# bioinformatics-centre/kaiju

Measured on AMD Instinct MI355X. Metric: classified reads/sec (150 bp), higher is better.
Workload: dtype u64

## Files before the change

kaiju_amd/csrc/capi.hip:

```cpp
#include <hip/hip_runtime.h>
#include <fcntl.h>
#include <sys/stat.h>
#include <time.h>
#include <unistd.h>

#include <algorithm>
#include <atomic>
#include <cstdio>
#include <cstring>
#include <future>
#include <memory>
#include <mutex>
#include <stdexcept>
#include <string>
#include <thread>
#include <vector>
#include <chrono>

#include "../../include/kaiju_gpu.h"
#include "fmi_stream.h"
#include "host_index.h"
#include "host_tables.h"
#include "kj_core.h"
#include "taxonomy.h"
// ... 65 lines not shown

constexpr int kS1TeamBlock = 256;
constexpr int kS1TeamsPerBlock = kS1TeamBlock / (int)kS1TeamLanes;
__global__ void __launch_bounds__(kS1TeamBlock)
k_fragments_team(const Stage1Tables *__restrict__ g_t, Params p, Batch b, uint32_t *err) {
  __shared__ __attribute__((aligned(16))) Stage1Tables s_t;
  __shared__ __attribute__((aligned(16))) S1TeamLds s_team[kS1TeamsPerBlock];
  {
    const uint4 *src = reinterpret_cast<const uint4 *>(g_t);
    uint4 *dst = reinterpret_cast<uint4 *>(&s_t);
    for (uint32_t i = threadIdx.x; i < sizeof(Stage1Tables) / 16; i += kS1TeamBlock) dst[i] = src[i];
    __syncthreads();
  }
  const uint32_t team = threadIdx.x / kS1TeamLanes;
  const uint32_t r = blockIdx.x * kS1TeamsPerBlock + team;
  if (r >= b.n_reads) return;
  uint32_t e = 0;
  S1TeamDev tm{&s_team[team], threadIdx.x % kS1TeamLanes};
  build_fragments_team(s_t, p, b, r, &e, tm);
  if (e) atomicOr(err, e);
}

__global__ void __launch_bounds__(256)
k_trigcheck(const Stage1Tables *__restrict__ g_t, Params p, Batch b, uint32_t *seglist, uint32_t *segcount) {
  __shared__ __attribute__((aligned(16))) Stage1Tables s_t;
  __shared__ __attribute__((aligned(4))) uint8_t s_cnt[256 * kS1CntStride];
  {
    const uint4 *src = reinterpret_cast<const uint4 *>(g_t);
    uint4 *dst = reinterpret_cast<uint4 *>(&s_t);
    for (uint32_t i = threadIdx.x; i < sizeof(Stage1Tables) / 16; i += 256) dst[i] = src[i];
    __syncthreads();
  }
  const uint32_t r = blockIdx.x * 256 + threadIdx.x;
  if (r >= b.n_reads) return;
  const uint32_t v = b.hits[r].reserved;
  if (v == 0) return;
  b.hits[r].reserved = 0;
  const bool need = lazy_seg_needed(s_t, p, b, r, b.hits + r, v, nullptr, s_cnt + threadIdx.x * kS1CntStride);
  if (need) seglist[atomicAdd(segcount, 1u)] = r;
}
__global__ void __launch_bounds__(256)
k_segflag(Params p, SegTables st, Batch b, SegQueue sq, const uint32_t *seglist, const uint32_t *segcount, uint32_t *err) {
  __shared__ int64_t s_entg[13];
  if (threadIdx.x < 13) s_entg[threadIdx.x] = st.ent_g[threadIdx.x];
  __syncthreads();
  const SegCtx cx = seg_ctx(st, s_entg, nullptr);
  const uint32_t n = *segcount;
  for (uint32_t i = blockIdx.x * 256 + threadIdx.x; i < n; i += gridDim.x * 256) {
    const uint32_t r = seglist[i];
    const ReadMeta rm = b.meta[r];
    Frag *F = b.frags + rm.frag;
    const uint8_t *pep = b.pep + rm.pep;
    const uint32_t nf = rm.nfrag & ~kNfragSegPending;
    uint32_t pending = 0;
    for (uint32_t k = 0; k < nf; k++) {
      const Frag f = F[k];
      uint32_t fl = kFragChecked;
      if (seg_triggers(cx, pep + f.start, (int)f.len)) {
        const uint32_t slot = atomicAdd(sq.count, 1u);
        if (slot >= sq.cap) atomicOr(err, 2u);
        else {
          SegWork wk; wk.read = r; wk.frag = k;
          sq.items[slot] = wk;
          pending = kNfragSegPending;
          fl = (slot + 1) << kFragSlotShift;
        }
      }
      F[k].flags = fl;
    }
    b.meta[r].nfrag = nf | pending;
    uint64_t *h8 = reinterpret_cast<uint64_t *>(b.hits + r);
    for (int x = 0; x < (int)(sizeof(Hit) / 8); x++) h8[x] = 0;
  }
}
__global__ void __launch_bounds__(kBlock)
k_seg_apply_list(const ConstTables *__restrict__ g_ct, Params p, Batch b, SegQueue sq, const uint32_t *seglist,
                 const uint32_t *segcount, uint32_t *err) {
  __shared__ ConstTables s_ct;
  load_tables(s_ct, g_ct);
  const uint32_t n = *segcount;
  uint32_t e = 0;
  for (uint32_t i = blockIdx.x * kBlock + threadIdx.x; i < n; i += gridDim.x * kBlock) seg_apply_mem(s_ct, p, b, sq, seglist[i], &e);
  if (e) atomicOr(err, e);
}

#ifdef KJ_POST_WAVES
#define KJ_POST_BOUNDS __launch_bounds__(256, KJ_POST_WAVES)
#else
#define KJ_POST_BOUNDS __launch_bounds__(256)
#endif
template <bool LCA>
__global__ void KJ_POST_BOUNDS
k_mem_post1(const Stage1Tables *__restrict__ g_t, DevIndex ix, Params p, Batch b, DevTaxonomy t, CompactHit *__restrict__ compact, int lazy,
            uint32_t *seglist, uint32_t *segcount, uint32_t *todo, uint32_t *todocount) {
  __shared__ __attribute__((aligned(16))) Stage1Tables s_t;
  __shared__ __attribute__((aligned(4))) uint8_t s_cnt[256 * kS1CntStride];
  if (lazy) {
    const uint4 *src = reinterpret_cast<const uint4 *>(g_t);
    uint4 *dst = reinterpret_cast<uint4 *>(&s_t);
    for (uint32_t i = threadIdx.x; i < sizeof(Stage1Tables) / 16; i += 256) dst[i] = src[i];
    __syncthreads();
  }
  const uint32_t r = blockIdx.x * 256 + threadIdx.x;
  bool need = false, later = false;
  if (r < b.n_reads) {
    Hit *h = b.hits + r;
    const uint32_t v = lazy ? h->reserved : 0u;
    if (v != 0) {
      h->reserved = 0;
#ifndef KJ_POST_NOTRIG
      need = lazy_seg_needed(s_t, p, b, r, h, v, nullptr, s_cnt + threadIdx.x * kS1CntStride);
#endif
    }
    if (!need) {
      if (h->flags & kHitRetry) later = true;
#ifdef KJ_POST_NOLOCATE
      else if (LCA) { CompactHit ch; ch.lca = 0; ch.best = h->best; ch.info = 0; compact[r] = ch; }
#else
      else if (!mem_locate_read<false>(ix, p, h, kLocDeferRows)) later = true;
      else if (LCA) compact[r] = compact_hit(t, *h);
#endif
    }
  }
  const uint32_t lane = threadIdx.x & 63u;
  {
    const uint64_t m = __ballot(need);
    if (m) {
      const uint32_t leader = (uint32_t)__builtin_ctzll(m);
      uint32_t base = 0;
      if (lane == leader) base = atomicAdd(segcount, (uint32_t)__popcll(m));
      base = (uint32_t)__shfl((int)base, (int)leader, 64);
      if (need) seglist[base + (uint32_t)__popcll(m & ((1ull << lane) - 1ull))] = r;
    }
  }
// ... 1501 lines not shown
  Params kp{};
  hipStream_t stream = nullptr;
  hipEvent_t ev[6] = {nullptr, nullptr, nullptr, nullptr, nullptr, nullptr};
  bool ev_valid = false;
  int n_cu = 0, blocks_main = 0, blocks_retry = 0;
  DevBuf pep, frags, meta, counters, retry_list, seg_items, seg_recs;
  DevBuf scratch_main[10], scratch_retry[5], h_compact;
  DevBuf redo_bitmap, redo_list, redo_items, redo_index, redo_pool, redo_work, redo_cls;
  bool greedy2 = false;
  bool greedy3 = false;
  uint32_t g3_split = 1;
  uint32_t g3_threads = 512;
  uint32_t g1_pool = 192, g1_match = 64;
  bool g1_pool_set = false;
  uint32_t greedy_gate = 1u | 32u << 8;
  bool verbose = false;
  bool exact_pass = true;
  bool count_ops = false;
  bool mem_v1 = false;
  bool verbose_v1 = false;
  bool stage1_old = false;
  bool stage1_lane = false;
  bool lazy_seg = true;
  DevBuf seglist, loc_list, todo_list;
  int seg_team = 64;
  bool fused_post = true;
  const char *dump_frags = nullptr;
  uint32_t vb_text_cap = 0;
  DevBuf vb_nacc, vb_acc, vb_tlen, vb_text, vb_bestv, vb_bestv_retry;
  DevBuf vb_packed, vb_pos;
  std::vector<uint8_t> vb_host;
  std::vector<uint32_t> vb_h_nacc, vb_h_acc;
  DevBuf h_seqs, h_off, h_hits;
  kj_ingest_scratch *ingest = nullptr;
  DevBuf ing_text1, ing_text2, ing_names, ing_info;
  kaiju_gpu_stats stats{};
  uint32_t last_n = 0;
  uint32_t max_read_len = 1024;
  ~kaiju_gpu_ctx() {
    if (!ix) return;
    (void)hipSetDevice(ix->device);
    if (ingest) kj_ingest_free(ingest);
    DevBuf *all[] = {&ing_text1, &ing_text2, &ing_names, &ing_info, &pep, &frags, &meta, &counters, &retry_list, &seg_items, &seg_recs, &h_seqs, &h_off, &h_hits, &h_compact, &seglist, &loc_list, &todo_list,
                     &vb_nacc, &vb_acc, &vb_tlen, &vb_text, &vb_bestv, &vb_bestv_retry, &vb_packed, &vb_pos,
                     &redo_bitmap, &redo_list, &redo_items, &redo_index, &redo_pool, &redo_work, &redo_cls};
    for (DevBuf *b : all) if (b->p) (void)hipFree(b->p);
// ... 33 lines not shown
  if (!out || !ix || !p) return fail(KAIJU_GPU_ERR_ARG, "NULL argument");
  *out = nullptr;
  if (p->mode != 0 && p->mode != 1) return fail(KAIJU_GPU_ERR_ARG, "mode must be 0 (MEM) or 1 (GREEDY)");
  if (p->min_fragment_length < 1 || p->min_fragment_length > 10000)
    return fail(KAIJU_GPU_ERR_UNSUPPORTED, "min_fragment_length out of range");
  if (p->mode == 1 && p->mismatches > (uint32_t)kMaxMismatch)
    return fail(KAIJU_GPU_ERR_UNSUPPORTED, "more than 8 mismatches are not supported");
  if (p->mode == 1 && p->seed_length < 1) return fail(KAIJU_GPU_ERR_ARG, "seed_length must be >= 1");
  if (p->max_match_ids > 20 || p->max_matches_SI > 64 || p->max_matches_SI < 1)
    return fail(KAIJU_GPU_ERR_UNSUPPORTED, "max_match_ids <= 20 and 1 <= max_matches_SI <= 64 required");
  std::unique_ptr<kaiju_gpu_ctx> c(new kaiju_gpu_ctx());
  c->ix = ix;
  c->params = *p;
  c->kp.mode = p->mode; c->kp.m = p->min_fragment_length; c->kp.mismatches = p->mismatches;
  c->kp.min_score = p->min_score; c->kp.seed_length = p->seed_length; c->kp.seg = p->seg ? 1 : 0;
  c->kp.max_matches_SI = p->max_matches_SI; c->kp.max_match_ids = p->max_match_ids;
  if (const char *e = getenv("KAIJU_GPU_DEBUG")) c->kp.debug = (uint32_t)atoi(e);
  if (const char *e = getenv("KAIJU_GPU_EXACT_PASS")) c->exact_pass = atoi(e) != 0;
  if (const char *e = getenv("KAIJU_GPU_MEM_LANE")) c->mem_v1 = !strcmp(e, "v1");
  if (const char *e = getenv("KAIJU_GPU_VERBOSE_LANE")) c->verbose_v1 = !strcmp(e, "v1");
  c->dump_frags = getenv("KAIJU_GPU_DUMP_FRAGS");
  if (const char *e = getenv("KAIJU_GPU_STAGE1")) { c->stage1_old = !strcmp(e, "old"); c->stage1_lane = !strcmp(e, "lane"); }
  if (const char *e = getenv("KAIJU_GPU_LAZY_SEG")) c->lazy_seg = atoi(e) != 0;
  if (const char *e = getenv("KAIJU_GPU_FUSED_POST")) c->fused_post = atoi(e) != 0;
  if (const char *e = getenv("KAIJU_GPU_SEG_TEAM")) { const int v = atoi(e); if (v == 8 || v == 16 || v == 32 || v == 64) c->seg_team = v; }
  if (ix->id_mode == KAIJU_GPU_IDS_SEQUENCE && p->mode == 0) c->kp.flags |= kParamXOrder;
  if (p->input_is_protein) c->kp.flags |= kParamProtein;
  KJ_HIP(hipSetDevice(ix->device));
  hipDeviceProp_t prop;
  KJ_HIP(hipGetDeviceProperties(&prop, ix->device));
  c->n_cu = prop.multiProcessorCount;
  int occ = 0;
  if (p->mode == 0) KJ_HIP(hipOccupancyMaxActiveBlocksPerMultiprocessor(&occ, k_mem, kBlock, 0));
  else {
    const bool g_wide = ix->dev.mb_base != nullptr;
    const uint32_t g_k = g_wide ? ix->dev.kmer_k : ix->dev.kline_k;
    c->greedy2 = ix->dev.blocks64 && (g_wide ? ix->dev.kmer64 != nullptr : ix->dev.kline != nullptr) && g_k >= 2 &&
                 g_k <= p->seed_length && p->seed_length >= 3;
    if (const char *e = getenv("KAIJU_GPU_GREEDY_LANE")) { if (!strcmp(e, "v1")) c->greedy2 = false; }
#ifdef KJ_GREEDY3
    if (const char *e = getenv("KAIJU_GPU_GREEDY_LANE")) { if (!strcmp(e, "v3")) c->greedy3 = c->greedy2 && !g_wide; }
    if (const char *e = getenv("KAIJU_GPU_G3_SPLIT")) c->g3_split = (uint32_t)atoi(e);
    if (const char *e = getenv("KAIJU_GPU_G3_THREADS")) { const int v = atoi(e); if (v >= 64 && v <= kG3Threads && v % 64 == 0) c->g3_threads = (uint32_t)v; }
#else
    if (const char *e = getenv("KAIJU_GPU_GREEDY_LANE")) {
      if (!strcmp(e, "v3")) return fail(KAIJU_GPU_ERR_UNSUPPORTED, "KAIJU_GPU_GREEDY_LANE=v3: this library was built without -DKJ_GREEDY3 (tests/tools/mem_variants.sh, variant g3)");
// ... 196 lines not shown
      const bool xo = (p.flags & kParamXOrder) != 0;
      SIEntry *si_main = static_cast<SIEntry *>(c->scratch_main[0].p);
      auto launch_v2 = [&](const Params &pp, const WorkList &wl, bool counting, bool second = false) {
        if (c->verbose) {
          if (mem_narrow2) hipLaunchKernelGGL(k_mem_vb, dim3(c->blocks_main), blk, 0, s, ix->dev, pp, b, wl, si_main, si_cap, vb.acc);
          else hipLaunchKernelGGL(k_mem_wide2_vb, dim3(c->blocks_main), blk, 0, s, ix->dev, pp, b, wl, si_main, si_cap, vb.acc);
        } else
        if (mem_narrow2) {
          if (second && !xo) hipLaunchKernelGGL(k_mem_second, dim3(c->blocks_main), blk, 0, s, ix->dev, pp, b, wl, si_main, si_cap);
          else if (counting) hipLaunchKernelGGL(k_mem_count, dim3(c->blocks_main), blk, 0, s, ix->dev, pp, b, wl, si_main, si_cap);
          else if (xo) hipLaunchKernelGGL(k_mem_x, dim3(c->blocks_main), blk, 0, s, ix->dev, pp, b, wl, si_main, si_cap);
          else hipLaunchKernelGGL(k_mem, dim3(c->blocks_main), blk, 0, s, ix->dev, pp, b, wl, si_main, si_cap);
        } else {
          if (counting) hipLaunchKernelGGL(k_mem_wide2_count, dim3(c->blocks_main), blk, 0, s, ix->dev, pp, b, wl, si_main, si_cap);
          else if (xo) hipLaunchKernelGGL(k_mem_wide2_x, dim3(c->blocks_main), blk, 0, s, ix->dev, pp, b, wl, si_main, si_cap);
          else hipLaunchKernelGGL(k_mem_wide2, dim3(c->blocks_main), blk, 0, s, ix->dev, pp, b, wl, si_main, si_cap);
        }
      };
      const bool defer = mem_v2;
      Params pd = p;
      if (defer) pd.flags |= kParamDeferLocate;
      if (mem_v2) {
        Params pm = pd;
        if (lazy) pm.flags |= kParamLazySeg;
        launch_v2(pm, wl_main, c->count_ops);
      } else if (!ix->dev.mb_base)
        hipLaunchKernelGGL(k_mem_v1, dim3(c->blocks_main), blk, 0, s, ix->dev, p, b, wl_main, si_main, si_cap, vb);
      else
        hipLaunchKernelGGL(k_mem_wide, dim3(c->blocks_main), blk, 0, s, ix->dev, p, b, wl_main, si_main, si_cap, vb);
      KJ_HIP(hipGetLastError());
      KJ_HIP(hipEventRecord(c->ev[3], s));
      uint32_t *todo = nullptr;
      const DevTaxonomy dt = tax ? tax->dev : DevTaxonomy{};
      CompactHit *const cmp = reinterpret_cast<CompactHit *>(d_compact);
      if (fused) {
        if ((rc = ensure(c->seglist, (size_t)n * 4 + 16))) return rc;
        if ((rc = ensure(c->todo_list, (size_t)n * 4 + 16))) return rc;
        todo = static_cast<uint32_t *>(c->todo_list.p);
        uint32_t *seglist = static_cast<uint32_t *>(c->seglist.p);
        if (tax) hipLaunchKernelGGL(k_mem_post1<true>, grid_reads, dim3(256), 0, s, ix->d_s1, ix->dev, p, b, dt, cmp, lazy ? 1 : 0, seglist, cnt + 22, todo, cnt + 26);
        else hipLaunchKernelGGL(k_mem_post1<false>, grid_reads, dim3(256), 0, s, ix->d_s1, ix->dev, p, b, dt, cmp, lazy ? 1 : 0, seglist, cnt + 22, todo, cnt + 26);
        KJ_HIP(hipGetLastError());
      }
      if (lazy) {
        if ((rc = ensure(c->seglist, (size_t)n * 4 + 16))) return rc;
        uint32_t *seglist = static_cast<uint32_t *>(c->seglist.p);
        if (!fused) hipLaunchKernelGGL(k_trigcheck, grid_reads, dim3(256), 0, s, ix->d_s1, p, b, seglist, cnt + 22);
        hipLaunchKernelGGL(k_segflag, dim3(c->n_cu * 4), dim3(256), 0, s, p, ix->st, b, sq, seglist, cnt + 22, cnt + 3);
        launch_seg(c, s, p, ix->st, b, sq);
        hipLaunchKernelGGL(k_seg_apply_list, dim3(c->n_cu * 4), blk, 0, s, ix->d_ct, p, b, sq, seglist, cnt + 22, cnt + 3);
        WorkList wl_seg;
        wl_seg.counter = cnt + 23; wl_seg.reads = seglist; wl_seg.n_items_ptr = cnt + 22; wl_seg.n_items = 0;
        wl_seg.retry_list = wl_main.retry_list; wl_seg.retry_count = wl_main.retry_count;
        launch_v2(pd, wl_seg, false, true);
        KJ_HIP(hipGetLastError());
      }
      hipLaunchKernelGGL(k_mem_retry, dim3(blocks_retry), blk, 0, s, ix->dev, p, b, wl_retry,
                         static_cast<SIEntry *>(c->scratch_retry[0].p), si_cap_retry, vb);
      KJ_HIP(hipGetLastError());
      if (defer && c->verbose) {
        if (mem_narrow2) hipLaunchKernelGGL(k_mem_verbose<false>, grid_reads, dim3(256), 0, s, ix->dev, p, b, vb);
        else hipLaunchKernelGGL(k_mem_verbose<true>, grid_reads, dim3(256), 0, s, ix->dev, p, b, vb);
        KJ_HIP(hipGetLastError());
      }
      if (defer && !fused) {
        if (mem_narrow2 && ix->dev.row_tax) {
          hipLaunchKernelGGL(k_mem_locate<false>, grid_reads, dim3(256), 0, s, ix->dev, p, b, loc_list, cnt + 24);
          hipLaunchKernelGGL(k_mem_locate_list<false>, dim3(c->n_cu * 8), dim3(256), 0, s, ix->dev, p, b, loc_list, cnt + 24);
        }
        else if (mem_narrow2) hipLaunchKernelGGL(k_mem_locate_team, grid_team, dim3(256), 0, s, ix->dev, p, b);
        else if (ix->dev.row_tax) {
// ... 755 lines not shown
```

kaiju_amd/csrc/kj_core.h:

```cpp
#pragma once
#include <type_traits>
#include <stdint.h>

#if defined(__HIPCC__)
#include <hip/hip_runtime.h>
#define KJ_HD __host__ __device__ __forceinline__
#define KJ_HD_NOINLINE __host__ __device__ __noinline__
#else
#define KJ_HD inline
#define KJ_HD_NOINLINE inline
struct uint2 { uint32_t x, y; };
struct ulonglong2 { uint64_t x, y; };
#endif

namespace kj {

struct u128 { uint64_t x, y; };
typedef u128 u128_unaligned __attribute__((aligned(1)));
typedef uint32_t u32_unaligned __attribute__((aligned(1)));
typedef uint64_t u64_unaligned __attribute__((aligned(1)));

constexpr int kMaxIds = 21;
constexpr int kSbShift = 16;
constexpr uint32_t kHitIdCap = 1u, kHitSiCap = 2u;
// ... 128 lines not shown
      {d.seq_valid, (uint64_t)d.nseq},
      {d.kmer32 ? (const void *)d.kmer32 : (const void *)d.kmer64, d.kmer_k ? nw * (d.kmer32 ? sizeof(uint2) : sizeof(ulonglong2)) : 0},
      {d.kline, d.kline ? nlw * kKLineBytes : 0},
      {d.text, d.text ? text_bytes : 0},
      {d.sa_full ? (const void *)d.sa_full : (const void *)d.sa_tpos5, d.sa_full ? d.bwtlen * 4 : d.sa_tpos5 ? tpos_bytes : 0},
      {d.row_tax, d.row_tax ? d.bwtlen * 4 : 0},
      {d.tax_of_dense, d.tax_of_dense ? (uint64_t)d.n_dense * 8 : 0}};
  for (int x = 0; x < kIndexArrays; x++) { out[x] = a[x]; if (!out[x].p || !out[x].bytes) out[x] = IndexArr{nullptr, 0}; }
}

struct Params {
  int32_t mode;
  uint32_t m;
  uint32_t mismatches, min_score, seed_length;
  int32_t seg;
  uint32_t max_matches_SI, max_match_ids;
  uint32_t debug = 0;
  uint32_t flags = 0;
};
constexpr uint32_t kParamDeferLocate = 8u;
constexpr uint32_t kParamXOrder = 1u;
constexpr uint32_t kParamProtein = 2u;
constexpr uint32_t kParamLazySeg = 4u;
constexpr uint32_t kWinMulti = 0x80000000u;
constexpr uint32_t kWinForce = 0xffffffffu;

struct Frag {
  uint32_t start;
  uint32_t len;
  uint32_t key;
  uint32_t flags;
};

struct SegWork { uint32_t read, frag; };
constexpr int kSegRecRegions = 15;
struct SegRec {
  uint16_t n;
  uint16_t overflow;
  uint16_t lr[kSegRecRegions][2];
};
static_assert(sizeof(SegRec) == 64, "SegRec is 64 bytes");
struct SegQueue {
  SegWork *items;
  SegRec *recs;
  uint32_t *count;
  uint32_t cap;
};
constexpr uint32_t kFragChecked = 1u, kFragRemoved = 2u, kFragSlotShift = 8;
constexpr uint32_t kNfragSegPending = 0x80000000u;

struct SIEntry {
  uint64_t lo;
  uint32_t len;
  uint32_t frag;
};

struct Hit {
// ... 22 lines not shown
  uint8_t subst_rank[20][20];
  uint8_t codon_idx[64];
};

struct ReadMeta {
  uint64_t pep;
  uint32_t frag;
  uint32_t nfrag;
};

struct Batch {
  const uint8_t *seqs;
  const uint64_t *off;
  uint32_t n_reads;
  int32_t paired;
  uint8_t *pep;
  Frag *frags;
  ReadMeta *meta;
  Hit *hits;
};

constexpr uint64_t kPepPerRead = 208;
static_assert(kPepPerRead >= 2 * 96 + 15 + 1, "kPepPerRead must cover the unit padding of build_fragments_fast plus the rounding of pep_base");
KJ_HD uint64_t pep_base(const uint64_t *off, uint32_t r) { return ((2 * off[2 * (uint64_t)r] + 15) & ~15ull) + kPepPerRead * r + 16; }
KJ_HD uint64_t frag_base(const uint64_t *off, uint32_t r, uint32_t m) {
  return 2 * ((2 * off[2 * (uint64_t)r]) / (m + 1) + 7ull * r);
}
KJ_HD uint32_t frag_cap(const uint64_t *off, uint32_t r, uint32_t m) {
  return (uint32_t)(frag_base(off, r + 1, m) - frag_base(off, r, m));
}

KJ_HD uint32_t popc64(uint64_t x) { return (uint32_t)__builtin_popcountll(x); }

#if defined(__HIP_DEVICE_COMPILE__)
KJ_HD uint64_t kj_ballot(bool p) { return __ballot(p); }
KJ_HD uint32_t kj_lane() { return threadIdx.x & 63u; }
KJ_HD uint32_t kj_bcast(uint32_t v, uint32_t src_lane) { return (uint32_t)__shfl((int)v, (int)src_lane, 64); }
KJ_HD uint32_t kj_rank_below(uint64_t mask) {
  return __builtin_amdgcn_mbcnt_hi((uint32_t)(mask >> 32), __builtin_amdgcn_mbcnt_lo((uint32_t)mask, 0u));
}
KJ_HD uint32_t kj_bcast_uniform(uint32_t v, uint32_t src_lane) {
  return (uint32_t)__builtin_amdgcn_readlane((int)v, (int)__builtin_amdgcn_readfirstlane((int)src_lane));
}
KJ_HD uint32_t kj_alignbyte(uint32_t hi, uint32_t lo, uint32_t s) { return __builtin_amdgcn_alignbyte(hi, lo, s); }
#else
KJ_HD uint32_t kj_alignbyte(uint32_t hi, uint32_t lo, uint32_t s) { return (uint32_t)((((uint64_t)hi << 32) | lo) >> (8u * (s & 3u))); }
KJ_HD uint64_t kj_ballot(bool p) { return p ? 1ull : 0ull; }
// ... 626 lines not shown
    pep.put(base + (uint32_t)g * fcap + nres, 0);
    emit_run(p, list, n, cap, rbase + (uint32_t)g * fcap, R_len[g], R_sum[g], R_pend[g], R_trig[g]);
    pep.put(rbase + (uint32_t)g * fcap + nres, 0);
  }
}

template <class S>
KJ_HD bool seg_triggers(const SegCtx &cx, const S &s, int len) {
  if (len < kSegWindow) return false;
  SegWin w{0, 0, 0};
  segwin_open(w, cx, s, 0);
  if (w.score <= cx.ent_locut) return true;
  for (int start = 0; start + kSegWindow < len; start++) {
    segwin_shift(w, cx, s, start);
    if (w.score <= cx.ent_locut) return true;
  }
  return false;
}

template <class Coop, class Sync>
KJ_HD void seg_compute(const SegCtx &cx, const Coop &coop, const Batch &b, const Params &p, const SegQueue &sq,
                       uint32_t slot, uint8_t *stage, uint32_t stage_cap, int32_t *work, uint8_t *cls, Sync &&team_sync) {
  const SegWork wk = sq.items[slot];
  const ReadMeta rm = b.meta[wk.read];
  const Frag f = b.frags[rm.frag + wk.frag];
  const uint8_t *pep = b.pep + rm.pep;
  const uint8_t *src = pep + f.start;
  if (stage && f.len <= stage_cap) {
    team_sync();
    for (uint32_t x = (uint32_t)coop.lane(); x < f.len; x += (uint32_t)coop.width()) stage[x] = src[x];
    team_sync();
    src = stage;
  }
  int32_t *left = work + 2 * kSegMaxRegions, *right = work + 3 * kSegMaxRegions;
  bool ov = false;
  const int n = seg_regions(cx, coop, src, (int)f.len, left, right, ov, work, (stage && f.len <= stage_cap) ? cls : nullptr, team_sync);
  if (coop.lane() != 0) return;
  SegRec rec;
  rec.overflow = (ov || n > kSegRecRegions || f.len > 65535u) ? 1 : 0;
  rec.n = (uint16_t)(n > kSegRecRegions ? kSegRecRegions : n);
  for (int k = 0; k < kSegRecRegions; k++) {
    rec.lr[k][0] = k < n ? (uint16_t)left[k] : 0;
    rec.lr[k][1] = k < n ? (uint16_t)right[k] : 0;
  }
  sq.recs[slot] = rec;
}

template <class Sink>
KJ_HD void seg_split(const ConstTables &t, const Params &p, const SegRec &rec, const uint8_t *pep,
                     const Frag &f, Sink &&sink) {
// ... 86 lines not shown
  const uint64_t pbase = pep_base(b.off, r);
  PepBuf pep;
  if (stage) { pep.base = stage; pep.row = stage_row; } else { pep.base = b.pep + pbase; pep.row = 4; }
  uint32_t n = 0, pending = 0;
  const bool skip = b.paired ? (len1 < m3 && len2 < m3) : (len1 < m3);
  if (!skip) {
    const uint32_t seq2 = 2 * len1 + 6, seq_end = seq2 + 2 * len2 + 6;
    if (len1 >= m3) translate_mate(t, p, tc, b.seqs + o0, len1, 0, pep, 0, list, n, cap);
    if (b.paired && len2 >= m3) translate_mate(t, p, tc, b.seqs + o1, len2, seq2, pep, 6 * (len1 / 3 + 1), list, n, cap);
    if (stage && !(p.debug & 8u)) {
      const uint32_t used = 6 * (len1 / 3 + 1) + (b.paired ? 6 * (len2 / 3 + 1) : 0);
      u128 *dst = reinterpret_cast<u128 *>(b.pep + pbase);
      for (uint32_t q = 0; q * 16 < used; q++) {
        u128 v;
        v.x = (uint64_t)pep.get32(16 * q) | (uint64_t)pep.get32(16 * q + 4) << 32;
        v.y = (uint64_t)pep.get32(16 * q + 8) | (uint64_t)pep.get32(16 * q + 12) << 32;
        dst[q] = v;
      }
    }
    if (p.debug & 16u) n = 0;
    uint32_t sb = 1;
    while ((1u << sb) <= seq_end) sb++;
    const uint32_t kbound = 11u * ((len1 > len2 ? len1 : len2) / 3u + 1u);
    auto final_flags = [&](uint32_t trig, uint32_t k) -> uint32_t {
      if (!p.seg) return 0u;
      if (!trig) return kFragChecked;
      const uint32_t slot = append_slot(sq.count);
      if (slot >= sq.cap) { if (err_flags) *err_flags |= 2u; return kFragChecked; }
      SegWork wk; wk.read = r; wk.frag = k;
      sq.items[slot] = wk;
      pending = kNfragSegPending;
      return (slot + 1) << kFragSlotShift;
    };
    if (stage && n <= stage_words / 2 && sb <= 20 && kbound < (1u << (31 - sb))) {
      uint32_t *row = reinterpret_cast<uint32_t *>(stage);
      const uint32_t rw = stage_row / 4, half = stage_words / 2, smax = (1u << sb) - 1u;
      for (uint32_t k0 = 0; k0 < n; k0 += 4) {
        Frag f[4];
#pragma unroll
        for (int x = 0; x < 4; x++) f[x] = list[k0 + (uint32_t)x < n ? k0 + (uint32_t)x : k0];
#pragma unroll
        for (int x = 0; x < 4; x++) {
          const uint32_t k = k0 + (uint32_t)x;
          if (k < n) {
            row[(size_t)k * rw] = f[x].key << (sb + 1) | (smax - (f[x].flags >> 1)) << 1 | (f[x].flags & 1u);
            row[(size_t)(half + k) * rw] = f[x].start << 16 | f[x].len;
          }
        }
      }
      for (uint32_t k = 0; k < n; k++) {
        const uint32_t ck = row[(size_t)k * rw];
        uint32_t rank = 0;
        for (uint32_t q = 0; q < n; q++) rank += row[(size_t)q * rw] > ck ? 1u : 0u;
        const uint32_t sl = row[(size_t)(half + k) * rw];
        Frag f; f.start = sl >> 16; f.len = sl & 0xffffu; f.key = ck >> (sb + 1); f.flags = final_flags(ck & 1u, rank);
        list[rank] = f;
      }
    } else {
      for (uint32_t k = 1; k < n; k++) {
        const Frag f = list[k];
        uint32_t pos = k;
        while (pos > 0 && (list[pos - 1].key < f.key || (list[pos - 1].key == f.key && list[pos - 1].flags > f.flags))) {
          list[pos] = list[pos - 1]; pos--;
        }
        list[pos] = f;
      }
      for (uint32_t k = 0; k < n; k++) list[k].flags = final_flags(list[k].flags & 1u, k);
    }
  }
  ReadMeta rm; rm.pep = pbase; rm.frag = (uint32_t)frag_base(b.off, r, p.m); rm.nfrag = n | pending;
  b.meta[r] = rm;
}

struct Stage1Tables {
  uint8_t nuc3[256];
  uint8_t tf[512];
  uint8_t tr[512];
  int32_t dtab[32];
  uint8_t diag[32];
  int32_t locut32;
  int32_t pad[3];
};
static_assert(sizeof(Stage1Tables) % 16 == 0, "Stage1Tables is copied in 16-byte pieces");
constexpr int kS1Units = 4;
constexpr uint32_t kS1MaxLen = 48 * kS1Units - 1;
constexpr int kS1UnitsLong = 6;
constexpr uint32_t kS1MaxLenLong = 48 * kS1UnitsLong - 1;
struct Mask128 { uint64_t lo, hi; };
KJ_HD uint64_t mk_zero(uint64_t) { return 0; }
KJ_HD Mask128 mk_zero(Mask128) { return Mask128{0, 0}; }
KJ_HD void mk_or16(uint64_t &m, uint32_t bits, uint32_t b) { m |= (uint64_t)bits << (16u * b); }
KJ_HD void mk_or16(Mask128 &m, uint32_t bits, uint32_t b) { if (b < 4u) m.lo |= (uint64_t)bits << (16u * b); else m.hi |= (uint64_t)bits << (16u * (b - 4u)); }
KJ_HD void mk_setbit(uint64_t &m, uint32_t k, bool v) { m |= (uint64_t)(v ? 1u : 0u) << k; }
KJ_HD void mk_setbit(Mask128 &m, uint32_t k, bool v) { if (k < 64u) m.lo |= (uint64_t)(v ? 1u : 0u) << k; else m.hi |= (uint64_t)(v ? 1u : 0u) << (k - 64u); }
KJ_HD bool mk_any(uint64_t m) { return m != 0; }
KJ_HD bool mk_any(const Mask128 &m) { return (m.lo | m.hi) != 0; }
KJ_HD uint64_t mk_shr(uint64_t m, uint32_t n) { return m >> n; }
KJ_HD Mask128 mk_shr(const Mask128 &m, uint32_t n) {
  if (n == 0u) return m;
  if (n >= 128u) return Mask128{0, 0};
  if (n >= 64u) return Mask128{m.hi >> (n - 64u), 0};
  return Mask128{(m.lo >> n) | (m.hi << (64u - n)), m.hi >> n};
}
KJ_HD uint64_t mk_shl(uint64_t m, uint32_t n) { return m << n; }
KJ_HD Mask128 mk_shl(const Mask128 &m, uint32_t n) {
  if (n == 0u) return m;
  if (n >= 128u) return Mask128{0, 0};
  if (n >= 64u) return Mask128{0, m.lo << (n - 64u)};
  return Mask128{m.lo << n, (m.hi << n) | (m.lo >> (64u - n))};
}
// ... 195 lines not shown
      sc += same ? 0 : dx - dy;
      any = any || sc <= t.locut32;
    }
#pragma unroll
    for (int q = 0; q < 4; q++) pw[q] = w[q];
  }
  return any;
}
KJ_HD bool lazy_seg_needed(const Stage1Tables &t, const Params &p, const Batch &b, uint32_t r, const Hit *h, uint32_t v, uint8_t *buf, uint8_t *row) {
  if (v == kWinForce) return true;
  const ReadMeta rm = b.meta[r];
  const Frag *F = b.frags + rm.frag;
  const uint8_t *pep = b.pep + rm.pep;
  if (!(v & kWinMulti)) {
    const Frag f = F[(v & ~kWinMulti) - 1u];
    return buf ? trig_fragment(t, pep, f.start, f.len, buf, row) : trig_fragment_units(t, pep, f.start, f.len, row);
  }
  const uint32_t best = h->best, nf = rm.nfrag & ~kNfragSegPending;
  for (uint32_t k = 0; k < nf; k++) {
    const Frag f = F[k];
    if (f.len >= best && (buf ? trig_fragment(t, pep, f.start, f.len, buf, row) : trig_fragment_units(t, pep, f.start, f.len, row))) return true;
  }
  return false;
}
KJ_HD uint64_t bitrev64(uint64_t v) {
#if defined(__HIP_DEVICE_COMPILE__)
  return __brevll(v);
#else
  uint64_t r = 0;
  for (int i = 0; i < 64; i++) r |= ((v >> i) & 1ull) << (63 - i);
  return r;
#endif
}

KJ_HD uint64_t mk_rev_low(uint64_t m, uint32_t nbits) { return bitrev64(m) >> (64u - nbits); }
KJ_HD Mask128 mk_rev_low(const Mask128 &m, uint32_t nbits) { return mk_shr(Mask128{bitrev64(m.hi), bitrev64(m.lo)}, 128u - nbits); }

KJ_HD uint32_t s1_start(int f, uint32_t u, uint32_t a, uint32_t l) {
  return f < 3 ? (uint32_t)f * (16 * u) + a : (uint32_t)(f + 1) * (16 * u) - a - l;
}

template <class MaskT, class Emit>
KJ_HD void s1_runs(const MaskT *ns, const MaskT *tg, uint32_t len, uint32_t m, uint32_t area, uint32_t seq_base,
                   Emit &&emit) {
  if (m > 64u || m == 0u) return;
  const uint32_t top = len - 3, u = len / 48u + 1u;
// ... 69 lines not shown
    MaskT ns[6], tg[6];
    for (int f = 0; f < 6; f++) tg[f] = mk_zero(MaskT{});
    auto scan_mate = [&](uint8_t *dst, uint32_t len) {
      const uint32_t u = len / 48u + 1u;
      for (int f = 0; f < 6; f++) {
        const MaskT mm = trig_scan_units<UNITS, MaskT>(t, dst + (size_t)f * 16 * u, u, ln.cnt);
        const MaskT tv = f < 3 ? mm : mk_shl(mk_rev_low(mm, 16 * u), 11);
#pragma unroll
        for (int q = 0; q < 6; q++) if (q == f) tg[q] = tv;
      }
    };
    if (len1 >= m3) {
      s1_mate(t, b.seqs + o0, len1, area, ns);
#ifndef KJ_S1_NOSCAN
      if (TRIG && p.seg) scan_mate(area, len1);
#endif
      s1_runs(ns, tg, len1, p.m, 0, 0, emit);
    }
    if (b.paired && len2 >= m3) {
      s1_mate(t, b.seqs + o1, len2, area + mate_bytes, ns);
      if (TRIG && p.seg) scan_mate(area + mate_bytes, len2);
      s1_runs(ns, tg, len2, p.m, mate_bytes, 2 * len1 + 6, emit);
    }
    auto final_flags = [&](uint32_t trig, uint32_t k) -> uint32_t {
      if (!TRIG || !p.seg) return 0u;
      if (!trig) return kFragChecked;
      const uint32_t slot = append_slot(sq.count);
      if (slot >= sq.cap) { if (err_flags) *err_flags |= 2u; return kFragChecked; }
      SegWork wk; wk.read = r; wk.frag = k;
      sq.items[slot] = wk;
      pending = kNfragSegPending;
      return (slot + 1) << kFragSlotShift;
    };
    if (n <= (uint32_t)kS1ListCap) {
      for (uint32_t k = 0; k < n; k++) {
        const uint32_t hi = ln.codes[(size_t)(2 * k) * ln.code_stride], lo = ln.codes[(size_t)(2 * k + 1) * ln.code_stride];
        uint32_t rank = 0;
        for (uint32_t q = 0; q < n; q++) rank += ln.codes[(size_t)(2 * q) * ln.code_stride] > hi ? 1u : 0u;
        Frag f; f.start = lo >> 8; f.len = (lo >> 1) & 127u; f.key = hi >> 11; f.flags = final_flags(lo & 1u, rank);
        list[rank] = f;
      }
    } else {
      for (uint32_t k = 0; k < (uint32_t)kS1ListCap; k++) {
        const uint32_t hi = ln.codes[(size_t)(2 * k) * ln.code_stride], lo = ln.codes[(size_t)(2 * k + 1) * ln.code_stride];
        Frag f; f.start = lo >> 8; f.len = (lo >> 1) & 127u; f.key = hi >> 11; f.flags = (2047u - (hi & 2047u)) << 1 | (lo & 1u);
        list[k] = f;
      }
      for (uint32_t k = 1; k < n; k++) {
        const Frag f = list[k];
        uint32_t pos = k;
        while (pos > 0 && (list[pos - 1].key < f.key || (list[pos - 1].key == f.key && list[pos - 1].flags > f.flags))) {
          list[pos] = list[pos - 1]; pos--;
        }
        list[pos] = f;
      }
      for (uint32_t k = 0; k < n; k++) list[k].flags = final_flags(list[k].flags & 1u, k);
    }
  }
  ReadMeta rm; rm.pep = pbase; rm.frag = fbase; rm.nfrag = n | pending;
  b.meta[r] = rm;
}

constexpr uint32_t kS1TeamLanes = 16;
struct S1TeamLds {
  u128 str[6 * kS1Units];
  uint64_t ns[6];
  uint32_t hi[kS1ListCap], lo[kS1ListCap];
  uint32_t n, pad[3];
};
static_assert(sizeof(S1TeamLds) % 16 == 0, "S1TeamLds is an array of 16-byte aligned team areas");

struct S1TeamHost {
  static constexpr int kSlots = (int)kS1TeamLanes;
  S1TeamLds *lds;
  KJ_HD uint32_t lane(int s) const { return (uint32_t)s; }
  KJ_HD void sync() const {}
  KJ_HD void sync_memory() const {}
  KJ_HD uint32_t xor1(const uint32_t *v, int s) const { return v[s ^ 1]; }
  KJ_HD uint32_t dword(const uint8_t *s, uint32_t len, int32_t at) const {
// ... 237 lines not shown
        emit_run(p, list, n, cap, run_start, run_len, sum, seq++, trig);
        run_len = 0; sum = 0; trig = false;
        trig_reset(w);
      }
    }
    *reinterpret_cast<uint64_t *>(pep + (len & ~7u)) = wacc;
    emit_run(p, list, n, cap, run_start, run_len, sum, seq, trig);
    for (uint32_t k = 1; k < n; k++) {
      const Frag f = list[k];
      uint32_t pos = k;
      while (pos > 0 && (list[pos - 1].key < f.key || (list[pos - 1].key == f.key && list[pos - 1].flags > f.flags))) {
        list[pos] = list[pos - 1]; pos--;
      }
      list[pos] = f;
    }
    for (uint32_t k = 0; k < n; k++) {
      uint32_t fl = 0;
      if (p.seg) {
        fl = kFragChecked;
        if (list[k].flags & 1u) {
          const uint32_t slot = append_slot(sq.count);
          if (slot >= sq.cap) { if (err_flags) *err_flags |= 2u; }
          else {
            SegWork wk; wk.read = r; wk.frag = k;
            sq.items[slot] = wk;
            pending = kNfragSegPending;
            fl = (slot + 1) << kFragSlotShift;
          }
        }
      }
      list[k].flags = fl;
    }
  }
  ReadMeta rm; rm.pep = pbase; rm.frag = (uint32_t)frag_base(b.off, r, p.m); rm.nfrag = n | pending;
  b.meta[r] = rm;
}

KJ_HD void seg_apply_mem(const ConstTables &t, const Params &p, const Batch &b, const SegQueue &sq, uint32_t r,
                         uint32_t *err_flags) {
  const ReadMeta rm = b.meta[r];
  const uint32_t raw = rm.nfrag;
  if (!(raw & kNfragSegPending)) return;
  const uint32_t n_orig = raw & ~kNfragSegPending;
  Frag *list = b.frags + rm.frag;
  const uint32_t cap = frag_cap(b.off, r, p.m);
  const uint8_t *pep = b.pep + rm.pep;
  uint32_t np = 0;
  for (uint32_t k = 0; k < n_orig; k++) {
// ... 700 lines not shown
    if (parked) kind = kind_saved;
    KJ_PM(PM_TAIL);
    {
      if (bk == BK_END_MATCH) {
        KJ_PM(PM_END_MATCH);
        const uint32_t l = (uint32_t)(j - i + 1);
        KJ_HIST_SINGLE_END(l);
        if constexpr (kSpanEq) last_sz = hi > lo ? (P)(hi - lo) : (P)1;
        bool probed = false;
        if constexpr (WIDE) {
          if (pj >= 0) {
            probed = true;
            if (l < pw) { j--; pj = -1; }
            else { j = pj; pj = -2; i = flen; }
            bk = BK_START_J;
          }
        }
        if (probed) {}
        else
        if (l >= L) {
          if (l > L) { nsi = 0; ovf = false; L = l; multi = false; }
          const uint32_t ilen = (uint32_t)(int32_t)(hi - lo);
          if (nsi != 0 && fcur != s0frag) multi = true;
          if constexpr (VERBOSE) { if (nsi < (uint32_t)kVbMem) ls.vbm[(size_t)r * kVbAcc + nsi] = fcur << 16 | ((uint32_t)i & 0xffffu); }
          if (nsi == 0) { s0lo = lo; s0len = ilen; s0frag = fcur; }
          else if (nsi == 1) { s1lo = lo; s1len = ilen; s1frag = fcur; }
          else if (nsi < ls.si_cap) { SIEntry e; e.lo = lo; e.len = ilen; e.frag = fcur; ls.si[nsi] = e; if constexpr (COUNT) oc[kOpcSiSpill]++; }
          else ovf = true;
          nsi++;
          found = true;
        }
        if (probed) {}
        else if (i <= 1) bk = BK_NEXT_FRAG;
        else { j--; bk = BK_START_J; }
      }
      if (bk == BK_START_J) {
        KJ_PM(PM_START_J);
        if (!WIDE && skipj && j >= (int)L - 1) {
          if (j <= 1) bk = BK_NEXT_FRAG; else j--;
        }
        skipj = false;
        if (bk == BK_NEXT_FRAG) {}
        else if (j < (int)L - 1 && !(WIDE && pj >= 0)) bk = BK_NEXT_FRAG;
        else if (kk && j >= (int)kk - 1) {
          if constexpr (WIDE) {
            if (kMemProbe && pj == -1 && L > pw) { pj = j; j -= (int)(L - pw); }
          }
// ... 4 lines not shown
              kidx = 0;
              for (uint32_t q = 0; q < kk; q++) kidx = kmer_index(kidx, lw.w[j - (int)q - lw.q]);
            } else {
              kidx = 0;
              for (uint32_t q = 1; q < kk; q++) kidx = kline_code(kidx, lw.w[e - (int)q - lw.q]);
              kidx = kline_ref(kidx, lw.w[e - lw.q]);
            }
            kind = probe ? K_PROBE : K_KMER; bk = BK_NONE;
            if (WIDE && pj == -2) pj = -1;
          } else { fill_top = j; fill_newfrag = false; fill_step = false; kind = K_FILL; bk = BK_NONE; }
        } else if (in_win(j)) {
          c = lw.w[j - lw.q];
          lo = (P)ix.C[c]; hi = (P)ix.C[c + 1];
          i = j;
          if (i == 0) bk = BK_END_MATCH;
          else if (in_win(i - 1)) { c = lw.w[i - 1 - lw.q]; kind = K_STEP; bk = BK_NONE; }
          else { fill_top = i - 1; fill_newfrag = false; fill_step = true; kind = K_FILL; bk = BK_NONE; }
        } else { fill_top = j; fill_newfrag = false; fill_step = false; kind = K_FILL; bk = BK_NONE; }
      }
      if (bk == BK_NEXT_FRAG) {
        KJ_PM(PM_NEXT_FRAG);
        if (f >= nf || (found && dnext.key < L)) bk = BK_LOC_INIT;
        else {
          fcur = f; f++;
          skipj = false;
          fsoff = pepoff + dnext.start; flen = (int)dnext.len;
          j = flen - 1;
          i = flen;
          pj = -1;
          fill_top = j; fill_newfrag = true; fill_step = false;
          kind = K_FILL; bk = BK_NONE;
        }
      }
      if (bk == BK_LOC_INIT) {
        KJ_PM(PM_LOC_INIT);
        nids = 0; flags = 0;
        hit->best = found ? L : 0u;
        hit->reserved = ((p.flags & kParamLazySeg) && found) ? (ovf ? kWinForce : ((s0frag + 1u) | (multi ? kWinMulti : 0u))) : 0u;
        if (!found) bk = BK_FINISH;
        else if (ovf) {
          if (p.flags & kParamLazySeg) flags = kHitRetry;
          else if (wl.retry_list) { wl.retry_list[append_slot(wl.retry_count)] = r; flags = kHitRetry; }
          else flags = kHitInternalOverflow;
          bk = BK_FINISH;
        } else if (nsi <= 2u && (!WIDE || (s0len < kLocWideMaxLen && (nsi < 2u || s1len < kLocWideMaxLen)))) {
          const bool swap = !XORDER && nsi == 2u && s0frag == s1frag;
          const uint64_t e0 = WIDE ? ((uint64_t)s0lo | (uint64_t)s0len << kLocWideShift) : ((uint64_t)(uint32_t)s0lo | (uint64_t)s0len << 32);
          const uint64_t e1 = WIDE ? ((uint64_t)s1lo | (uint64_t)s1len << kLocWideShift) : ((uint64_t)(uint32_t)s1lo | (uint64_t)s1len << 32);
          hit->taxid[0] = swap ? e1 : e0;
          if (nsi == 2u) hit->taxid[1] = swap ? e0 : e1;
          nids = nsi; flags = kHitLocPending;
          bk = BK_FINISH;
        } else {
          bool big = false;
          if constexpr (WIDE) for (uint32_t e = 0; e < nsi; e++) big = big || si_len(e) >= kLocWideMaxLen;
          if (big || nsi > (uint32_t)kMaxIds) {
            if (p.flags & kParamLazySeg) flags = kHitRetry;
            else if (wl.retry_list) { wl.retry_list[append_slot(wl.retry_count)] = r; flags = kHitRetry; }
            else flags = kHitInternalOverflow;
          } else {
            uint32_t q = 0, gs = 0;
// ... 1926 lines not shown
```

Baseline: 479.4 million.

## Carry fragment placement in hit and seg queue to skip meta/frag lookups

```diff
diff --git a/kaiju_amd/csrc/capi.hip b/kaiju_amd/csrc/capi.hip
--- a/kaiju_amd/csrc/capi.hip
+++ b/kaiju_amd/csrc/capi.hip
@@ -111,7 +111,7 @@
 }
 
 __global__ void __launch_bounds__(256)
-k_trigcheck(const Stage1Tables *__restrict__ g_t, Params p, Batch b, uint32_t *seglist, uint32_t *segcount) {
+k_trigcheck(const Stage1Tables *__restrict__ g_t, Params p, Batch b, int place, uint32_t *seglist, uint32_t *segcount) {
   __shared__ __attribute__((aligned(16))) Stage1Tables s_t;
   __shared__ __attribute__((aligned(4))) uint8_t s_cnt[256 * kS1CntStride];
   {
@@ -122,14 +122,16 @@
   }
   const uint32_t r = blockIdx.x * 256 + threadIdx.x;
   if (r >= b.n_reads) return;
+  const uint64_t off_2r = place ? b.off[2 * (uint64_t)r] : 0ull;
   const uint32_t v = b.hits[r].reserved;
   if (v == 0) return;
   b.hits[r].reserved = 0;
-  const bool need = lazy_seg_needed(s_t, p, b, r, b.hits + r, v, nullptr, s_cnt + threadIdx.x * kS1CntStride);
+  uint8_t *const row = s_cnt + threadIdx.x * kS1CntStride;
+  const bool need = place ? lazy_seg_needed_place(s_t, p, b, r, off_2r, b.hits + r, v, nullptr, row) : lazy_seg_needed(s_t, p, b, r, b.hits + r, v, nullptr, row);
   if (need) seglist[atomicAdd(segcount, 1u)] = r;
 }
 __global__ void __launch_bounds__(256)
-k_segflag(Params p, SegTables st, Batch b, SegQueue sq, const uint32_t *seglist, const uint32_t *segcount, uint32_t *err) {
+k_segflag(Params p, SegTables st, Batch b, SegQueue sq, int place, const uint32_t *seglist, const uint32_t *segcount, uint32_t *err) {
   __shared__ int64_t s_entg[13];
   if (threadIdx.x < 13) s_entg[threadIdx.x] = st.ent_g[threadIdx.x];
   __syncthreads();
@@ -142,14 +144,17 @@
     const uint8_t *pep = b.pep + rm.pep;
     const uint32_t nf = rm.nfrag & ~kNfragSegPending;
     uint32_t pending = 0;
+    Frag fnext = F[0];
     for (uint32_t k = 0; k < nf; k++) {
-      const Frag f = F[k];
+      const Frag f = fnext;
+      if (k + 1u < nf) fnext = F[k + 1u];
       uint32_t fl = kFragChecked;
       if (seg_triggers(cx, pep + f.start, (int)f.len)) {
         const uint32_t slot = atomicAdd(sq.count, 1u);
         if (slot >= sq.cap) atomicOr(err, 2u);
         else {
-          SegWork wk; wk.read = r; wk.frag = k;
+          SegWork wk = seg_work(r, k, rm.pep + f.start, f.len);
+          if (!place) wk.place = 0;
           sq.items[slot] = wk;
           pending = kNfragSegPending;
           fl = (slot + 1) << kFragSlotShift;
@@ -194,11 +199,13 @@
   bool need = false, later = false;
   if (r < b.n_reads) {
     Hit *h = b.hits + r;
+    const uint64_t off_2r = (lazy & 2) ? b.off[2 * (uint64_t)r] : 0ull;
     const uint32_t v = lazy ? h->reserved : 0u;
     if (v != 0) {
       h->reserved = 0;
 #ifndef KJ_POST_NOTRIG
-      need = lazy_seg_needed(s_t, p, b, r, h, v, nullptr, s_cnt + threadIdx.x * kS1CntStride);
+      uint8_t *const row = s_cnt + threadIdx.x * kS1CntStride;
+      need = (lazy & 2) ? lazy_seg_needed_place(s_t, p, b, r, off_2r, h, v, nullptr, row) : lazy_seg_needed(s_t, p, b, r, h, v, nullptr, row);
 #endif
     }
     if (!need) {
@@ -1746,6 +1753,7 @@
   bool stage1_old = false;
   bool stage1_lane = false;
   bool lazy_seg = true;
+  bool lazy_place = true;
   DevBuf seglist, loc_list, todo_list;
   int seg_team = 64;
   bool fused_post = true;
@@ -1825,6 +1833,7 @@
   c->dump_frags = getenv("KAIJU_GPU_DUMP_FRAGS");
   if (const char *e = getenv("KAIJU_GPU_STAGE1")) { c->stage1_old = !strcmp(e, "old"); c->stage1_lane = !strcmp(e, "lane"); }
   if (const char *e = getenv("KAIJU_GPU_LAZY_SEG")) c->lazy_seg = atoi(e) != 0;
+  if (const char *e = getenv("KAIJU_GPU_LAZY_PLACE")) c->lazy_place = atoi(e) != 0;
   if (const char *e = getenv("KAIJU_GPU_FUSED_POST")) c->fused_post = atoi(e) != 0;
   if (const char *e = getenv("KAIJU_GPU_SEG_TEAM")) { const int v = atoi(e); if (v == 8 || v == 16 || v == 32 || v == 64) c->seg_team = v; }
   if (ix->id_mode == KAIJU_GPU_IDS_SEQUENCE && p->mode == 0) c->kp.flags |= kParamXOrder;
@@ -2067,7 +2076,7 @@
       if (defer) pd.flags |= kParamDeferLocate;
       if (mem_v2) {
         Params pm = pd;
-        if (lazy) pm.flags |= kParamLazySeg;
+        if (lazy) pm.flags |= kParamLazySeg | (c->lazy_place ? kParamLazyPlace : 0u);
         launch_v2(pm, wl_main, c->count_ops);
       } else if (!ix->dev.mb_base)
         hipLaunchKernelGGL(k_mem_v1, dim3(c->blocks_main), blk, 0, s, ix->dev, p, b, wl_main, si_main, si_cap, vb);
@@ -2083,15 +2092,16 @@
         if ((rc = ensure(c->todo_list, (size_t)n * 4 + 16))) return rc;
         todo = static_cast<uint32_t *>(c->todo_list.p);
         uint32_t *seglist = static_cast<uint32_t *>(c->seglist.p);
-        if (tax) hipLaunchKernelGGL(k_mem_post1<true>, grid_reads, dim3(256), 0, s, ix->d_s1, ix->dev, p, b, dt, cmp, lazy ? 1 : 0, seglist, cnt + 22, todo, cnt + 26);
-        else hipLaunchKernelGGL(k_mem_post1<false>, grid_reads, dim3(256), 0, s, ix->d_s1, ix->dev, p, b, dt, cmp, lazy ? 1 : 0, seglist, cnt + 22, todo, cnt + 26);
+        const int lazy_arg = lazy ? (c->lazy_place ? 3 : 1) : 0;
+        if (tax) hipLaunchKernelGGL(k_mem_post1<true>, grid_reads, dim3(256), 0, s, ix->d_s1, ix->dev, p, b, dt, cmp, lazy_arg, seglist, cnt + 22, todo, cnt + 26);
+        else hipLaunchKernelGGL(k_mem_post1<false>, grid_reads, dim3(256), 0, s, ix->d_s1, ix->dev, p, b, dt, cmp, lazy_arg, seglist, cnt + 22, todo, cnt + 26);
         KJ_HIP(hipGetLastError());
       }
       if (lazy) {
         if ((rc = ensure(c->seglist, (size_t)n * 4 + 16))) return rc;
         uint32_t *seglist = static_cast<uint32_t *>(c->seglist.p);
-        if (!fused) hipLaunchKernelGGL(k_trigcheck, grid_reads, dim3(256), 0, s, ix->d_s1, p, b, seglist, cnt + 22);
-        hipLaunchKernelGGL(k_segflag, dim3(c->n_cu * 4), dim3(256), 0, s, p, ix->st, b, sq, seglist, cnt + 22, cnt + 3);
+        if (!fused) hipLaunchKernelGGL(k_trigcheck, grid_reads, dim3(256), 0, s, ix->d_s1, p, b, c->lazy_place ? 1 : 0, seglist, cnt + 22);
+        hipLaunchKernelGGL(k_segflag, dim3(c->n_cu * 4), dim3(256), 0, s, p, ix->st, b, sq, c->lazy_place ? 1 : 0, seglist, cnt + 22, cnt + 3);
         launch_seg(c, s, p, ix->st, b, sq);
         hipLaunchKernelGGL(k_seg_apply_list, dim3(c->n_cu * 4), blk, 0, s, ix->d_ct, p, b, sq, seglist, cnt + 22, cnt + 3);
         WorkList wl_seg;
diff --git a/kaiju_amd/csrc/kj_core.h b/kaiju_amd/csrc/kj_core.h
--- a/kaiju_amd/csrc/kj_core.h
+++ b/kaiju_amd/csrc/kj_core.h
@@ -174,8 +174,13 @@
 constexpr uint32_t kParamXOrder = 1u;
 constexpr uint32_t kParamProtein = 2u;
 constexpr uint32_t kParamLazySeg = 4u;
+constexpr uint32_t kParamLazyPlace = 16u;
 constexpr uint32_t kWinMulti = 0x80000000u;
 constexpr uint32_t kWinForce = 0xffffffffu;
+constexpr uint32_t kWinLenShift = 16, kWinStartMax = 0xffffu, kWinLenMax = 0x7fffu;
+KJ_HD uint32_t win_place(uint32_t start, uint32_t len) {
+  return (start <= kWinStartMax && len <= kWinLenMax) ? (start | len << kWinLenShift) : (kWinMulti | start);
+}
 
 struct Frag {
   uint32_t start;
@@ -184,7 +189,14 @@
   uint32_t flags;
 };
 
-struct SegWork { uint32_t read, frag; };
+struct SegWork { uint32_t read, frag; uint64_t place = 0; };
+static_assert(sizeof(SegWork) == 16, "SegWork is 16 bytes");
+constexpr uint32_t kSegPlaceShift = 40, kSegPlaceMaxLen = 0xffffffu;
+KJ_HD SegWork seg_work(uint32_t read, uint32_t frag, uint64_t pep_off, uint32_t len) {
+  SegWork wk; wk.read = read; wk.frag = frag;
+  wk.place = pep_off | (uint64_t)(len < kSegPlaceMaxLen ? len : kSegPlaceMaxLen) << kSegPlaceShift;
+  return wk;
+}
 constexpr int kSegRecRegions = 15;
 struct SegRec {
   uint16_t n;
@@ -253,7 +265,8 @@
 
 constexpr uint64_t kPepPerRead = 208;
 static_assert(kPepPerRead >= 2 * 96 + 15 + 1, "kPepPerRead must cover the unit padding of build_fragments_fast plus the rounding of pep_base");
-KJ_HD uint64_t pep_base(const uint64_t *off, uint32_t r) { return ((2 * off[2 * (uint64_t)r] + 15) & ~15ull) + kPepPerRead * r + 16; }
+KJ_HD uint64_t pep_base_at(uint64_t off_2r, uint32_t r) { return ((2 * off_2r + 15) & ~15ull) + kPepPerRead * r + 16; }
+KJ_HD uint64_t pep_base(const uint64_t *off, uint32_t r) { return pep_base_at(off[2 * (uint64_t)r], r); }
 KJ_HD uint64_t frag_base(const uint64_t *off, uint32_t r, uint32_t m) {
   return 2 * ((2 * off[2 * (uint64_t)r]) / (m + 1) + 7ull * r);
 }
@@ -926,10 +939,14 @@
 KJ_HD void seg_compute(const SegCtx &cx, const Coop &coop, const Batch &b, const Params &p, const SegQueue &sq,
                        uint32_t slot, uint8_t *stage, uint32_t stage_cap, int32_t *work, uint8_t *cls, Sync &&team_sync) {
   const SegWork wk = sq.items[slot];
-  const ReadMeta rm = b.meta[wk.read];
-  const Frag f = b.frags[rm.frag + wk.frag];
-  const uint8_t *pep = b.pep + rm.pep;
-  const uint8_t *src = pep + f.start;
+  struct { uint32_t len; } f{(uint32_t)(wk.place >> kSegPlaceShift)};
+  const uint8_t *src = b.pep + (wk.place & ((1ull << kSegPlaceShift) - 1ull));
+  if (wk.place == 0) {
+    const ReadMeta rm = b.meta[wk.read];
+    const Frag fd = b.frags[rm.frag + wk.frag];
+    f.len = fd.len;
+    src = b.pep + rm.pep + fd.start;
+  }
   if (stage && f.len <= stage_cap) {
     team_sync();
     for (uint32_t x = (uint32_t)coop.lane(); x < f.len; x += (uint32_t)coop.width()) stage[x] = src[x];
@@ -1062,13 +1079,12 @@
     uint32_t sb = 1;
     while ((1u << sb) <= seq_end) sb++;
     const uint32_t kbound = 11u * ((len1 > len2 ? len1 : len2) / 3u + 1u);
-    auto final_flags = [&](uint32_t trig, uint32_t k) -> uint32_t {
+    auto final_flags = [&](uint32_t trig, uint32_t k, uint32_t start, uint32_t len) -> uint32_t {
       if (!p.seg) return 0u;
       if (!trig) return kFragChecked;
       const uint32_t slot = append_slot(sq.count);
       if (slot >= sq.cap) { if (err_flags) *err_flags |= 2u; return kFragChecked; }
-      SegWork wk; wk.read = r; wk.frag = k;
-      sq.items[slot] = wk;
+      sq.items[slot] = seg_work(r, k, pbase + start, len);
       pending = kNfragSegPending;
       return (slot + 1) << kFragSlotShift;
     };
@@ -1093,7 +1109,7 @@
         uint32_t rank = 0;
         for (uint32_t q = 0; q < n; q++) rank += row[(size_t)q * rw] > ck ? 1u : 0u;
         const uint32_t sl = row[(size_t)(half + k) * rw];
-        Frag f; f.start = sl >> 16; f.len = sl & 0xffffu; f.key = ck >> (sb + 1); f.flags = final_flags(ck & 1u, rank);
+        Frag f; f.start = sl >> 16; f.len = sl & 0xffffu; f.key = ck >> (sb + 1); f.flags = final_flags(ck & 1u, rank, f.start, f.len);
         list[rank] = f;
       }
     } else {
@@ -1105,7 +1121,7 @@
         }
         list[pos] = f;
       }
-      for (uint32_t k = 0; k < n; k++) list[k].flags = final_flags(list[k].flags & 1u, k);
+      for (uint32_t k = 0; k < n; k++) list[k].flags = final_flags(list[k].flags & 1u, k, list[k].start, list[k].len);
     }
   }
   ReadMeta rm; rm.pep = pbase; rm.frag = (uint32_t)frag_base(b.off, r, p.m); rm.nfrag = n | pending;
@@ -1126,6 +1142,8 @@
 constexpr uint32_t kS1MaxLen = 48 * kS1Units - 1;
 constexpr int kS1UnitsLong = 6;
 constexpr uint32_t kS1MaxLenLong = 48 * kS1UnitsLong - 1;
+static_assert(2u * 6u * 16u * (uint32_t)kS1UnitsLong <= kWinStartMax + 1u && 16u * (uint32_t)kS1UnitsLong <= kWinLenMax,
+              "a fragment's place behind the fast stage 1 fits Hit::reserved");
 struct Mask128 { uint64_t lo, hi; };
 KJ_HD uint64_t mk_zero(uint64_t) { return 0; }
 KJ_HD Mask128 mk_zero(Mask128) { return Mask128{0, 0}; }
@@ -1367,6 +1385,14 @@
     if (f.len >= best && (buf ? trig_fragment(t, pep, f.start, f.len, buf, row) : trig_fragment_units(t, pep, f.start, f.len, row))) return true;
   }
   return false;
+}
+KJ_HD bool lazy_seg_needed_place(const Stage1Tables &t, const Params &p, const Batch &b, uint32_t r, uint64_t off_2r, const Hit *h, uint32_t v,
+                                 uint8_t *buf, uint8_t *row) {
+  if (v == kWinForce) return true;
+  if (v & kWinMulti) return lazy_seg_needed(t, p, b, r, h, v, buf, row);
+  const uint8_t *pep = b.pep + pep_base_at(off_2r, r);
+  const uint32_t start = v & kWinStartMax, len = v >> kWinLenShift;
+  return buf ? trig_fragment(t, pep, start, len, buf, row) : trig_fragment_units(t, pep, start, len, row);
 }
 KJ_HD uint64_t bitrev64(uint64_t v) {
 #if defined(__HIP_DEVICE_COMPILE__)
@@ -1482,13 +1508,12 @@
       if (TRIG && p.seg) scan_mate(area + mate_bytes, len2);
       s1_runs(ns, tg, len2, p.m, mate_bytes, 2 * len1 + 6, emit);
     }
-    auto final_flags = [&](uint32_t trig, uint32_t k) -> uint32_t {
+    auto final_flags = [&](uint32_t trig, uint32_t k, uint32_t start, uint32_t len) -> uint32_t {
       if (!TRIG || !p.seg) return 0u;
       if (!trig) return kFragChecked;
       const uint32_t slot = append_slot(sq.count);
       if (slot >= sq.cap) { if (err_flags) *err_flags |= 2u; return kFragChecked; }
-      SegWork wk; wk.read = r; wk.frag = k;
-      sq.items[slot] = wk;
+      sq.items[slot] = seg_work(r, k, pbase + start, len);
       pending = kNfragSegPending;
       return (slot + 1) << kFragSlotShift;
     };
@@ -1497,7 +1522,7 @@
         const uint32_t hi = ln.codes[(size_t)(2 * k) * ln.code_stride], lo = ln.codes[(size_t)(2 * k + 1) * ln.code_stride];
         uint32_t rank = 0;
         for (uint32_t q = 0; q < n; q++) rank += ln.codes[(size_t)(2 * q) * ln.code_stride] > hi ? 1u : 0u;
-        Frag f; f.start = lo >> 8; f.len = (lo >> 1) & 127u; f.key = hi >> 11; f.flags = final_flags(lo & 1u, rank);
+        Frag f; f.start = lo >> 8; f.len = (lo >> 1) & 127u; f.key = hi >> 11; f.flags = final_flags(lo & 1u, rank, f.start, f.len);
         list[rank] = f;
       }
     } else {
@@ -1514,7 +1539,7 @@
         }
         list[pos] = f;
       }
-      for (uint32_t k = 0; k < n; k++) list[k].flags = final_flags(list[k].flags & 1u, k);
+      for (uint32_t k = 0; k < n; k++) list[k].flags = final_flags(list[k].flags & 1u, k, list[k].start, list[k].len);
     }
   }
   ReadMeta rm; rm.pep = pbase; rm.frag = fbase; rm.nfrag = n | pending;
@@ -1798,8 +1823,7 @@
           const uint32_t slot = append_slot(sq.count);
           if (slot >= sq.cap) { if (err_flags) *err_flags |= 2u; }
           else {
-            SegWork wk; wk.read = r; wk.frag = k;
-            sq.items[slot] = wk;
+            sq.items[slot] = seg_work(r, k, pbase + list[k].start, list[k].len);
             pending = kNfragSegPending;
             fl = (slot + 1) << kFragSlotShift;
           }
@@ -2546,7 +2570,7 @@
           if (l > L) { nsi = 0; ovf = false; L = l; multi = false; }
           const uint32_t ilen = (uint32_t)(int32_t)(hi - lo);
           if (nsi != 0 && fcur != s0frag) multi = true;
-          if constexpr (VERBOSE) { if (nsi < (uint32_t)kVbMem) ls.vbm[(size_t)r * kVbAcc + nsi] = fcur << 16 | ((uint32_t)i & 0xffffu); }
+          if constexpr (VERBOSE) { if (nsi < (uint32_t)kVbMem) ls.vbm[(size_t)r * kVbAcc + nsi] = (f - 1u) << 16 | ((uint32_t)i & 0xffffu); }
           if (nsi == 0) { s0lo = lo; s0len = ilen; s0frag = fcur; }
           else if (nsi == 1) { s1lo = lo; s1len = ilen; s1frag = fcur; }
           else if (nsi < ls.si_cap) { SIEntry e; e.lo = lo; e.len = ilen; e.frag = fcur; ls.si[nsi] = e; if constexpr (COUNT) oc[kOpcSiSpill]++; }
@@ -2597,7 +2621,8 @@
         KJ_PM(PM_NEXT_FRAG);
         if (f >= nf || (found && dnext.key < L)) bk = BK_LOC_INIT;
         else {
-          fcur = f; f++;
+          fcur = (p.flags & kParamLazyPlace) ? win_place(dnext.start, dnext.len) : f;
+          f++;
           skipj = false;
           fsoff = pepoff + dnext.start; flen = (int)dnext.len;
           j = flen - 1;
@@ -2611,7 +2636,7 @@
         KJ_PM(PM_LOC_INIT);
         nids = 0; flags = 0;
         hit->best = found ? L : 0u;
-        hit->reserved = ((p.flags & kParamLazySeg) && found) ? (ovf ? kWinForce : ((s0frag + 1u) | (multi ? kWinMulti : 0u))) : 0u;
+        hit->reserved = ((p.flags & kParamLazySeg) && found) ? (ovf ? kWinForce : ((s0frag + ((p.flags & kParamLazyPlace) ? 0u : 1u)) | (multi ? kWinMulti : 0u))) : 0u;
         if (!found) bk = BK_FINISH;
         else if (ovf) {
           if (p.flags & kParamLazySeg) flags = kHitRetry;
```

New measurement: 476.1 million. Within noise of the previous version (-0.7%).
